# YuanchenBei/ColdRec

Hardware: AMD Instinct MI355X
Metric: ranked items/sec (full-catalogue eval) (higher is better)
Workload: dtype f32; 1 GPU; configs[3] full-catalogue eval: 1000000-row user table x 10000000 items, d=128, k=20, f32 tables, user block 131072 per step, rated CSR (mean ~50) + 20% cold-item bitmap ('warm' setting), item table row-sharded over 1 GPU(s); items=10000000, dim=128, k=20, parallelism=single GPU

## Files before the change

coldrec_amd/_lib.py:

```python
from __future__ import annotations

import ctypes
import os
import subprocess

_HERE = os.path.dirname(os.path.abspath(__file__))
LIB_PATH = os.environ.get("CRH_LIB") or os.path.join(_HERE, "lib", "libcoldrec_hip.so")
CSRC = os.path.join(_HERE, "csrc")

PAD_IDX = 0x7FFFFFFF
MASKED_SCORE = -1.0e9
MAX_K = 128

_lib = None

_vp, _i32, _i64, _sz, _f32 = ctypes.c_void_p, ctypes.c_int, ctypes.c_int64, ctypes.c_size_t, ctypes.c_float
_f64 = ctypes.c_double

SIGNATURES = {
    "crh_last_error": (ctypes.c_char_p, []),
    "crh_version": (_i32, []),
    "crh_score_topk_supports_dim": (_i32, [_i32]),
    "crh_score_topk_workspace_bytes": (_sz, [_i64, _i64, _i32, _i32]),
    "crh_score_topk_min_workspace_bytes": (_sz, [_i64, _i32]),
    "crh_score_topk_route": (_i32, [_i32, _i64, _i64, _i32, _i32, _sz, _i32, _i32, _vp, _vp]),
    "crh_score_topk_route_kernel": (ctypes.c_char_p, [_i32]),
    "crh_score_topk_screened": (_i32, [_i32, _i64, _i64, _i32, _i32, _sz, _i32, _i32]),
    "crh_score_topk_uncertified": (_i64, [_vp, _vp]),
    "crh_score_topk_screen_plan": (_i32, [_i64, _i64, _sz, _i32, _vp, _vp]),
    "crh_score_topk_screen_ordered": (_i32, [_i64, _i64, _sz, _i32]),
    "crh_score_topk_screen_map": (_i32, [_vp, _vp, _i64, _i64, _i64, _i32, _vp, _vp, _vp, _vp]),
    "crh_score_topk_screen_rated_tiles": (_i32, [_i64, _i64, _sz, _i32, _i32]),
    "crh_score_topk_screen_flags_bytes": (_sz, [_i64, _i64]),
    "crh_score_topk_screen_flags": (_i32, [_vp, _vp, _i64, _i64, _i64, _i32, _vp, _vp, _i64, _vp, _vp]),
    "crh_score_topk_f32": (_i32, [_vp, _vp, _i64, _vp, _i64, _i32, _vp, _vp, _vp, _i32, _i64, _vp, _vp,
                                  _vp, _sz, _vp]),
    "crh_score_topk_f32_ex": (_i32, [_vp, _vp, _i64, _vp, _i64, _i32, _vp, _vp, _vp, _i32, _i64, _vp, _vp,
                                     _vp, _sz, _vp, _i32, _vp, _vp]),
    "crh_score_screen_items_bytes": (_sz, [_i64, _i32]),
    "crh_score_screen_items_prepare": (_i32, [_vp, _i64, _i32, _vp, _i64, _i64, _vp, _sz, _vp, _sz, _vp, _vp]),
    "crh_score_screen_items_destroy": (_i32, [_vp]),
    "crh_score_topk_screen_item_preps": (_i64, []),
    "crh_score_topk_f32_prepared": (_i32, [_vp, _vp, _i64, _vp, _i64, _i32, _vp, _vp, _vp, _i32, _i64, _vp, _vp,
                                           _vp, _sz, _vp, _i32, _vp, _vp, _vp]),
    "crh_score_topk_f16_supports_dim": (_i32, [_i32]),
    "crh_score_topk_f16_workspace_bytes": (_sz, [_i64, _i64, _i32, _i32]),
    "crh_score_topk_f16_ex": (_i32, [_vp, _vp, _i64, _vp, _i64, _i32, _vp, _vp, _vp, _i32, _i64, _vp, _vp,
                                     _vp, _sz, _vp, _i32, _vp, _vp]),
    "crh_mask_topk_f32": (_i32, [_vp, _i64, _i64, _i64, _vp, _vp, _vp, _i32, _i64, _i32, _vp, _vp, _vp]),
    "crh_merge_topk": (_i32, [_vp, _vp, _i32, _i64, _i32, _i32, _vp, _vp, _vp]),
    "crh_bpr_workspace_bytes": (_sz, [_i64]),
    "crh_bpr_plan_ints": (_i64, [_i64]),
    "crh_bpr_heavy_threshold": (_i32, []),
    "crh_bpr_plan_build_host": (_i32, [_vp, _vp, _vp, _i64, _i64, _vp]),
    "crh_bpr_plan_build": (_i32, [_vp, _vp, _vp, _i64, _i64, _vp, _vp]),
    "crh_bpr_plan_build_large_workspace_bytes": (_sz, [_i64, _i64]),
    "crh_bpr_plan_build_large": (_i32, [_vp, _vp, _vp, _i64, _i64, _vp, _vp, _sz, _vp]),
    "crh_bpr_fwd_bwd_f32": (_i32, [_vp, _vp, _vp, _i32, _vp, _vp, _vp, _i64, _f32, _vp, _vp, _vp, _vp, _vp, _vp,
                                   _sz, _vp]),
    "crh_bpr_fwd_f32": (_i32, [_vp, _vp, _vp, _i32, _vp, _vp, _vp, _i64, _vp, _vp, _sz, _vp]),
    "crh_bpr_bwd_f32": (_i32, [_vp, _vp, _vp, _i32, _vp, _vp, _vp, _i64, _i64, _f32, _vp, _vp, _vp, _vp, _vp, _vp,
# ... 162 lines not shown
```

coldrec_amd/csrc/score_screen.hip:

```cpp
#include <math.h>

#include "score_topk_common.h"

#include <hipcub/device/device_radix_sort.hpp>

namespace crh_score {
namespace {

constexpr int SD = 128;
constexpr int FB_SCRATCH_SLICES = 64;

__device__ __forceinline__ float up_float(double x) {
    if (!(x <= 3.0e38)) return __builtin_inff();
    float f = (float)x;
    if ((double)f < x) f = __uint_as_float(__float_as_uint(f) + 1u);
    return f;
}

__device__ __forceinline__ int scale_exp(const unsigned* stats, int word) {
    const float m = __uint_as_float(stats[word]);
    if (!(m > 0.0f) || !(m <= 3.4e38f)) return 0;
    int E;
    frexpf(m, &E);
    return 15 - E;
}

__device__ __forceinline__ _Float16 to_f16(float x, int e) {
    const float y = ldexpf(x, e);
    _Float16 hv = (_Float16)y;
    if (fabsf((float)hv) < 6.103515625e-05f) hv = (_Float16)0.0f;
    return hv;
}

__device__ __forceinline__ float wave_max(float v) {
#pragma unroll
    for (int o = 32; o >= 1; o >>= 1) v = fmaxf(v, __shfl_xor(v, o));
    return v;
}

constexpr unsigned SCREEN_KEY_NONFINITE = 0x7F80u;
template <bool KEYS>
__global__ __launch_bounds__(256) void screen_maxabs_kernel(const float* __restrict__ tab, const int32_t* __restrict__ rows,
                                                            int64_t n_rows, unsigned* __restrict__ stats, int word,
                                                            uint16_t* __restrict__ keys) {
    const int64_t n4 = n_rows * (SD / 4);
    float m = 0.0f;
    for (int64_t e = (int64_t)blockIdx.x * 256 + threadIdx.x; e < n4; e += (int64_t)gridDim.x * 256) {
        const int64_t r = e / (SD / 4);
// ... 283 lines not shown
}

__global__ __launch_bounds__(256) void screen_certify_kernel(ScreenArgs s) {
    const int lane = threadIdx.x & 63;
    const int64_t slot = (int64_t)blockIdx.x * 4 + (threadIdx.x >> 6);
    if (slot >= s.n_users) return;
    const int KP = s.kp, K = s.k;
    const bool mine = lane < KP;
    int gi = CRH_PAD_IDX;
    float a = CRH_NEG_INF;
    if (mine) {
        gi = s.cand_idx[slot * KP + lane];
        a = s.cand_score[slot * KP + lane];
    }
    const bool real = mine && gi != CRH_PAD_IDX && (int64_t)gi >= s.item_base && (int64_t)gi < s.item_base + s.n_items;
    bool masked = false;
    if (real && s.bitmap) masked = (s.bitmap[gi >> 5] >> (gi & 31)) & 1u;
    if (real && !masked && s.rated_rowptr) masked = lane_in_list(s.rated_col, s.rated_rowptr[slot], s.rated_rowptr[slot + 1], gi);
    const int64_t urow = s.users ? (int64_t)s.users[slot] : slot;
    float sc = CRH_NEG_INF;
    if (real) sc = exact_chain(s.user_emb + urow * SD, s.item_emb + ((int64_t)gi - s.item_base) * SD);
    const bool ok = !mine || (real && !masked && __builtin_isfinite(a) && __builtin_isfinite(sc));
    int rank = 0;
    for (int j = 0; j < KP; ++j) {
        const float sj = __shfl(sc, j);
        const int ij = __shfl(gi, j);
        rank += (j != lane && crh_better(sj, ij, sc, gi)) ? 1 : 0;
    }
    const unsigned long long kth = __ballot(mine && rank == K - 1);
    const float ek = __shfl(sc, kth ? __builtin_ctzll(kth) : 0);
    const float a_last = __shfl(a, KP - 1);
    const float a_k = __shfl(a, K - 1);
    bool cert = s.mode != 3 && __ballot(!ok) == 0ull && kth != 0ull;
    if (cert) {
        const float* us = s.ustat + 3 * slot;
        const float R = __uint_as_float(s.stats[2]), N = __uint_as_float(s.stats[3]), Nh = __uint_as_float(s.stats[4]);
        const double B = screen_bound(us[0], us[1], us[2], R, N, Nh);
        const double unscale = ldexp(1.0, -(scale_exp(s.stats, 0) + scale_exp(s.stats, 1)));
        const double A = (double)a_last * unscale;
        double thr = A + B;
        thr += fabs(thr) * 0x1p-50;
        cert = (double)ek > thr && ek > CRH_MASKED_SCORE;
        const float Mk = __uint_as_float(s.stats[SCREEN_STAT_MARGIN]);
        if (Mk <= 3.4028235e38f) {
            double thr_m = ((double)a_k - (double)Mk) * unscale + B;
            thr_m += fabs(thr_m) * 0x1p-50;
            cert = cert && (double)ek > thr_m;
        }
    }
    if (cert) {
        if (mine && rank < K) {
            s.out_score[slot * K + rank] = sc;
            s.out_idx[slot * K + rank] = gi;
        }
    } else if (lane == 0) {
        const unsigned f = atomicAdd(s.stats + 5, 1u);
        s.fail_list[f] = (int32_t)slot;
    }
}

constexpr int64_t FB_WAVES = 2048 * 4;
constexpr int64_t FB_MIN_ITEMS = 1024;
constexpr int FB_FANIN = 64;
constexpr int FB_SLICES_MAX = FB_FANIN * FB_FANIN;
__device__ __forceinline__ int fb_slices(const ScreenArgs& s, int64_t count) {
    if (count <= 0) return 1;
    int64_t S = (FB_WAVES + count - 1) / count;
    const int64_t by_items = (s.n_items + FB_MIN_ITEMS - 1) / FB_MIN_ITEMS;
    const int64_t by_scratch = s.n_users * s.n_slices / count;
    if (S > by_items) S = by_items;
    if (S > by_scratch) S = by_scratch;
    if (S > FB_SLICES_MAX) S = FB_SLICES_MAX;
    return S < 1 ? 1 : (int)S;
}

__global__ __launch_bounds__(256) void screen_fallback_kernel(ScreenArgs s) {
    __shared__ float ush[4][SD];
    __shared__ float lsh[4][32];
    __shared__ int lih[4][32];
    __shared__ int cnth[4];
    const int lane = threadIdx.x & 63, wv = threadIdx.x >> 6;
    const int K = s.k;
    const int64_t count = s.stats[5];
    const int S = fb_slices(s, count);
    const int64_t n_work = count * S;
    float* ls = lsh[wv];
    int* li = lih[wv];
    int* cnt = &cnth[wv];
    for (int64_t w = (int64_t)blockIdx.x * 4 + wv; w < n_work; w += (int64_t)gridDim.x * 4) {
        const int64_t f = w / S;
        const int z = (int)(w % S);
        const int64_t slot = s.fail_list[f];
        const int64_t urow = s.users ? (int64_t)s.users[slot] : slot;
        ush[wv][lane] = s.user_emb[urow * SD + lane];
        ush[wv][lane + 64] = s.user_emb[urow * SD + lane + 64];
        if (lane == 0) *cnt = 0;
        const int64_t lo = s.n_items * z / S, hi = s.n_items * (z + 1) / S;
        float tau = CRH_NEG_INF;
        for (int64_t base = lo; base < hi; base += 64) {
            const int64_t i = base + lane;
            const bool valid = i < hi;
            const int gl = (int)(s.item_base + (valid ? i : lo));
            const bool bm = valid && s.bitmap && ((s.bitmap[gl >> 5] >> (gl & 31)) & 1u);
            float raw = CRH_NEG_INF;
            if (valid) {
                if (bm) {
                    raw = 0.0f;
#pragma unroll 8
                    for (int q = 0; q < SD; ++q) raw = __builtin_fmaf(ush[wv][q], 0.0f, raw);
                } else {
                    raw = exact_chain(ush[wv], s.item_emb + i * SD);
                }
            }
            unsigned long long cand = __ballot(valid && raw > tau);
            const unsigned long long bms = __ballot(bm);
            while (cand) {
                const int L = __builtin_ctzll(cand);
                cand &= cand - 1;
                float sc = __shfl(raw, L);
                const int g = (int)(s.item_base + base + L);
                const int n = __builtin_amdgcn_readfirstlane(*cnt);
                if (wave_list_rejects(ls, li, n, K, sc, g)) continue;
                bool masked = (bms >> L) & 1ull;
                if (!masked && s.rated_rowptr) masked = wave_is_masked(g, slot, s.rated_rowptr, s.rated_col, nullptr, lane);
                if (masked) sc = CRH_MASKED_SCORE;
                wave_list_insert(ls, li, cnt, K, sc, g, lane);
                tau = wave_list_tau(ls, __builtin_amdgcn_readfirstlane(*cnt), K);
            }
        }
        const int n = __builtin_amdgcn_readfirstlane(*cnt);
        const int64_t o = (f * S + z) * K;
        wave_list_store(ls, li, n, K, s.part_score + o, s.part_idx + o, lane);
    }
}

__global__ __launch_bounds__(256) void screen_fallback_merge_kernel(ScreenArgs s, int level) {
    __shared__ float lsh[4][32];
    __shared__ int lih[4][32];
    __shared__ int cnth[4];
    const int lane = threadIdx.x & 63, wv = threadIdx.x >> 6;
    const int K = s.k;
    const int64_t count = s.stats[5];
    const int S = fb_slices(s, count);
    const int last = S <= FB_FANIN ? 0 : 1;
    if (level > last) return;
    const int stride = level == 0 ? 1 : FB_FANIN;
    const int span = stride * FB_FANIN;
    const int G = (S + span - 1) / span;
    float* ls = lsh[wv];
    int* li = lih[wv];
    int* cnt = &cnth[wv];
    for (int64_t w = (int64_t)blockIdx.x * 4 + wv; w < count * G; w += (int64_t)gridDim.x * 4) {
        const int64_t f = w / G;
        const int z0 = (int)(w % G) * span;
        if (lane == 0) *cnt = 0;
        for (int z = z0; z < z0 + span && z < S; z += stride) {
            const int64_t o = (f * S + z) * K;
            const float es = lane < K ? s.part_score[o + lane] : CRH_NEG_INF;
            const int ei = lane < K ? s.part_idx[o + lane] : CRH_PAD_IDX;
            unsigned long long m = __ballot(lane < K && ei != CRH_PAD_IDX);
            while (m) {
                const int L = __builtin_ctzll(m);
                m &= m - 1;
                const float sc = __shfl(es, L);
                const int g = __shfl(ei, L);
                const int n = __builtin_amdgcn_readfirstlane(*cnt);
                if (n >= K && !crh_better(sc, g, ls[K - 1], li[K - 1])) break;
                wave_list_insert(ls, li, cnt, K, sc, g, lane);
            }
        }
        const int n = __builtin_amdgcn_readfirstlane(*cnt);
        if (level == last) {
            const int64_t slot = s.fail_list[f];
            wave_list_store(ls, li, n, K, s.out_score + slot * K, s.out_idx + slot * K, lane);
        } else {
            const int64_t o = (f * S + z0) * K;
            wave_list_store(ls, li, n, K, s.part_score + o, s.part_idx + o, lane);
        }
    }
}

}

int screen_fallback_slices(int64_t n_items) {
    const int64_t s = n_items / 4096;
    return (int)(s < 1 ? 1 : (s > FB_SCRATCH_SLICES ? FB_SCRATCH_SLICES : s));
}

size_t screen_scan_bytes(int64_t n_main) { return (size_t)((n_main + 31) / 32 / LIVE_WPB + 2) * sizeof(unsigned); }

int64_t screen_map_slots(int64_t n_main) { return ((n_main + 31) / 32 + 1) * 32; }

size_t screen_sort_bytes(int64_t n_slots) { return (size_t)n_slots * 8 + ((size_t)1 << 20); }

int launch_screen_map(const uint32_t* bitmap, int64_t item_base, int64_t n_items, int64_t prefix, unsigned* n_live, unsigned* scan,
                      int32_t* idmap, const ScreenOrder* ord, hipStream_t st) {
    const int64_t g0 = item_base + prefix, g1 = item_base + n_items;
    const int64_t n_words = ((g1 - 1) >> 5) - (g0 >> 5) + 1, nb = (n_words + LIVE_WPB - 1) / LIVE_WPB;
    hipLaunchKernelGGL(screen_live_count_kernel, dim3((unsigned)nb), dim3(256), 0, st, bitmap, g0, g1, scan);
    CRH_HIP(hipGetLastError());
    hipLaunchKernelGGL(screen_live_scan_kernel, dim3(1), dim3(256), 0, st, scan, nb, n_live);
    CRH_HIP(hipGetLastError());
    hipLaunchKernelGGL(screen_idmap_kernel, dim3((unsigned)nb), dim3(256), 0, st, bitmap, g0, g1, scan, idmap);
    CRH_HIP(hipGetLastError());
    if (ord == nullptr) return CRH_OK;
    const int64_t n_slots = screen_map_slots(n_items - prefix);
    hipLaunchKernelGGL(screen_sortkey_kernel, dim3((unsigned)((n_slots + 255) / 256)), dim3(256), 0, st, idmap, ord->rowkeys, n_live,
                       item_base, n_slots, ord->skeys_in);
    CRH_HIP(hipGetLastError());
    size_t need = 0;
    CRH_HIP(hipcub::DeviceRadixSort::SortPairs(nullptr, need, ord->skeys_in, ord->skeys_out, idmap, ord->idmap, (int)n_slots, 0, 16, st));
    if (need > ord->sort_tmp_bytes) {
        crh_set_error("screened route: the ordered map's sort asks for %zu bytes of temporary storage, %zu are reserved", need,
                      ord->sort_tmp_bytes);
        return CRH_ERR_WS;
    }
    need = ord->sort_tmp_bytes;
    CRH_HIP(hipcub::DeviceRadixSort::SortPairs(ord->sort_tmp, need, ord->skeys_in, ord->skeys_out, idmap, ord->idmap, (int)n_slots, 0, 16, st));
    return CRH_OK;
// ... 72 lines not shown
    int32_t* idmap = reinterpret_cast<int32_t*>(buf + o_map);
    int rc = CRH_OK;
    unsigned live = 0;
    hipError_t e = hipMemsetAsync(buf, 0, 256, st);
    if (e == hipSuccess) {
        hipLaunchKernelGGL(screen_maxabs_kernel<true>, dim3(2048), dim3(256), 0, st, item_emb, nullptr, n_items, stats, 0, ord.rowkeys);
        e = hipGetLastError();
    }
    if (e == hipSuccess) rc = launch_screen_map(bitmap, item_base, n_items, prefix, stats + SCREEN_STAT_LIVE, reinterpret_cast<unsigned*>(buf + o_scan), idmap, &ord, st);
    if (e == hipSuccess && rc == CRH_OK) {
        hipLaunchKernelGGL(screen_mapkeys_kernel, dim3((unsigned)((n_main + 255) / 256)), dim3(256), 0, st,
                           ordered ? ord.skeys_out : ord.skeys_in, n_main, keys_out);
        e = hipGetLastError();
    }
    if (e == hipSuccess && rc == CRH_OK)
        e = hipMemcpyAsync(map_out, ordered ? ord.idmap : idmap, (size_t)n_main * 4, hipMemcpyDeviceToDevice, st);
    if (e == hipSuccess && rc == CRH_OK && flags_out != nullptr) {
        int32_t* inv = reinterpret_cast<int32_t*>(buf + o_inv);
        rc = launch_screen_invmap(ordered ? ord.idmap : idmap, stats + SCREEN_STAT_LIVE, item_base + prefix, n_main, inv, st);
        if (rc == CRH_OK)
            rc = launch_screen_rated_tiles(rated_rowptr, rated_col, n_users, bitmap, item_base + prefix, item_base + n_items, inv, flags_out, st);
    }
    if (e == hipSuccess && rc == CRH_OK) e = hipMemcpyAsync(&live, stats + SCREEN_STAT_LIVE, 4, hipMemcpyDeviceToHost, st);
    if (e == hipSuccess) e = hipStreamSynchronize(st);
    (void)hipFree(buf);
    CRH_HIP(e);
    if (rc == CRH_OK) *count = (int64_t)live;
    return rc;
}

int launch_screen_certify(const ScreenArgs& s, hipStream_t st) {
    hipLaunchKernelGGL(screen_certify_kernel, dim3((unsigned)((s.n_users + 3) / 4)), dim3(256), 0, st, s);
    CRH_HIP(hipGetLastError());
    hipLaunchKernelGGL(screen_fallback_kernel, dim3((unsigned)(FB_WAVES / 4)), dim3(256), 0, st, s);
    CRH_HIP(hipGetLastError());
    for (int level = 0; level < 2; ++level) {
        hipLaunchKernelGGL(screen_fallback_merge_kernel, dim3(512), dim3(256), 0, st, s, level);
        CRH_HIP(hipGetLastError());
    }
    return CRH_OK;
}

}
```

coldrec_amd/csrc/score_topk.hip:

```cpp
#include <math.h>
#include <stdarg.h>
#include <stdlib.h>

#include <algorithm>
#include <atomic>
#include <vector>

#include "score_topk_common.h"

using namespace crh_score;

namespace {

__device__ __forceinline__ bool pack_row_masked(const uint32_t* bitmap, int64_t gid) {
    return bitmap != nullptr && ((bitmap[gid >> 5] >> (gid & 31)) & 1u);
}

template <int D>
__global__ __launch_bounds__(256) void pack_items_kernel(const float* __restrict__ v, int64_t n_items,
                                                         float* __restrict__ packed, const uint32_t* __restrict__ bitmap,
                                                         int64_t item_base) {
    constexpr int NCH = D / 8;
    __shared__ float tile[32][D + 4];
    const int64_t t = blockIdx.x;
// ... 1245 lines not shown
    const int32_t* stream_map = nullptr;
    if (compact) stream_map = reuse ? reinterpret_cast<const int32_t*>(prepared->buf + PL.map) : (ordered ? ord.idmap : idmap);
    _Float16* uh = reinterpret_cast<_Float16*>(ws + L.uh);
    float* seed_s = reinterpret_cast<float*>(ws + L.seed);
    int32_t* seed_i = reinterpret_cast<int32_t*>(seed_s + (size_t)n_users * KP);
    float* cand_s = reinterpret_cast<float*>(ws + L.cand);
    int32_t* cand_i = reinterpret_cast<int32_t*>(cand_s + (size_t)n_users * KP);
    char* scratch = ws + L.scratch;
    const size_t scratch_b = workspace_bytes - L.scratch;

    ScreenArgs s;
    s.user_emb = user_emb;
    s.users = users;
    s.n_users = n_users;
    s.item_emb = item_emb;
    s.n_items = n_items;
    s.item_base = item_base;
    s.rated_rowptr = rated_rowptr;
    s.rated_col = rated_col;
    s.bitmap = cand_bitmap;
    s.k = k;
    s.kp = KP;
    s.mode = screen_mode();
    s.cand_score = cand_s;
    s.cand_idx = cand_i;
    s.stats = reinterpret_cast<unsigned*>(ws + L.stats);
    s.ustat = reinterpret_cast<float*>(ws + L.ustat);
    s.fail_list = reinterpret_cast<int32_t*>(ws + L.fail);
    s.n_slices = screen_fallback_slices(n_items);
    s.part_score = reinterpret_cast<float*>(scratch);
    s.part_idx = reinterpret_cast<int32_t*>(s.part_score + (size_t)n_users * s.n_slices * k);
    s.out_score = out_score;
    s.out_idx = out_idx;

    int rc = CRH_OK;
    if (reuse) {
        CRH_HIP(hipMemcpyAsync(s.stats, prepared->buf + PL.stats, 256, hipMemcpyDeviceToDevice, st));
    } else {
        CRH_HIP(hipMemsetAsync(s.stats, 0, 256, st));
        rc = screen_items_build(s, s.stats, pk, P, idmap, reinterpret_cast<unsigned*>(ws + L.scan), ordered ? &ord : nullptr, tbits, st);
        if (rc != CRH_OK) return rc;
    }
    const char* margin_env = getenv("CRH_SCORE_SCREEN_MARGIN");
    rc = launch_screen_prep_users(s, uh, !(margin_env && atoi(margin_env) == 0), st);
    if (rc != CRH_OK) return rc;
    if (ev_kernel_start) CRH_HIP(hipEventRecord(reinterpret_cast<hipEvent_t>(ev_kernel_start), st));

    ScoreArgs a = {};
    a.user_emb = uh;
    a.n_users = n_users;
    a.rated_rowptr = rated_rowptr;
    a.rated_col = rated_col;
    a.bitmap = cand_bitmap;
    a.k = KP;
    a.tile_bits = reinterpret_cast<const uint32_t*>(pk);
    if (P > 0) {
        const int64_t stride = P;
        const int upw_pw = users_per_wave(2, D);
        int64_t chunk = (int64_t)(scratch_b / ((size_t)stride * sizeof(float))) & ~(int64_t)63;
        if (chunk > n_users) chunk = n_users;
        a.packed = pk;
        a.n_items = P;
        a.item_base = item_base;
        a.dense = reinterpret_cast<float*>(scratch);
        a.dense_stride = stride;
        for (int64_t u0 = 0; u0 < n_users; u0 += chunk) {
// ... 235 lines not shown
    p->n_items = n_items;
    p->item_base = item_base;
    p->prefix = P;
    p->d = d;
    p->bitmap = cand_bitmap;
    p->compact = compact;
    p->ordered = ordered;
    p->stream = st;
    p->buf = buf;
    *handle = p;
    return CRH_OK;
}

extern "C" int crh_score_screen_items_destroy(void* handle) {
    if (handle == nullptr) return CRH_OK;
    ScreenItems* p = reinterpret_cast<ScreenItems*>(handle);
    CRH_CHECK_ARG(p->magic == SCREEN_ITEMS_MAGIC, "crh_score_screen_items_destroy: not a prepared-items handle");
    p->magic = 0;
    delete p;
    return CRH_OK;
}

extern "C" int64_t crh_score_topk_screen_item_preps(void) { return screen_item_preps.load(std::memory_order_relaxed); }

extern "C" int64_t crh_score_topk_uncertified(const void* workspace, void* stream) {
    CRH_CHECK_ARG(workspace != nullptr, "crh_score_topk_uncertified: NULL workspace");
    unsigned n = 0;
    hipStream_t st = reinterpret_cast<hipStream_t>(stream);
    CRH_HIP(hipMemcpyAsync(&n, reinterpret_cast<const unsigned*>(workspace) + 5, sizeof(n), hipMemcpyDeviceToHost, st));
    CRH_HIP(hipStreamSynchronize(st));
    return (int64_t)n;
}

extern "C" const char* crh_score_topk_route_kernel(int route) {
    switch (route & 15) {
        case CRH_ROUTE_DENSE: return "score_topk_kernel";
        case CRH_ROUTE_FUSED_WAVE: return "score_topk_kernel";
        case CRH_ROUTE_FUSED_WG: return "score_topk_wg_kernel";
        case CRH_ROUTE_FUSED_DMA: return "score_topk_dma_kernel";
        default: return "";
    }
}

extern "C" int crh_score_topk_f32_ex(const float* user_emb, const int32_t* users, int64_t n_users,
                                     const float* item_emb, int64_t n_items, int d,
                                     const int64_t* rated_rowptr, const int32_t* rated_col,
                                     const uint32_t* cand_bitmap, int k, int64_t item_base,
                                     float* out_score, int32_t* out_idx, void* workspace,
                                     size_t workspace_bytes, void* stream, int n_splits,
                                     void* ev_kernel_start, void* ev_kernel_stop) {
    return score_topk_any(4, user_emb, users, n_users, item_emb, n_items, d, rated_rowptr, rated_col, cand_bitmap, k,
                          item_base, out_score, out_idx, workspace, workspace_bytes, stream, n_splits,
                          ev_kernel_start, ev_kernel_stop, "crh_score_topk_f32");
}

extern "C" int crh_score_topk_f32_prepared(const float* user_emb, const int32_t* users, int64_t n_users,
                                           const float* item_emb, int64_t n_items, int d,
                                           const int64_t* rated_rowptr, const int32_t* rated_col,
                                           const uint32_t* cand_bitmap, int k, int64_t item_base,
                                           float* out_score, int32_t* out_idx, void* workspace,
                                           size_t workspace_bytes, void* stream, int n_splits,
                                           void* ev_kernel_start, void* ev_kernel_stop, const void* prepared) {
    return score_topk_any(4, user_emb, users, n_users, item_emb, n_items, d, rated_rowptr, rated_col, cand_bitmap, k,
                          item_base, out_score, out_idx, workspace, workspace_bytes, stream, n_splits,
                          ev_kernel_start, ev_kernel_stop, "crh_score_topk_f32", reinterpret_cast<const ScreenItems*>(prepared));
}
// ... 24 lines not shown
```

coldrec_amd/csrc/score_topk_common.h:

```cpp
#pragma once
#include <math.h>

#include "crh_common.h"
#include "topk_list.h"

namespace crh_score {

struct ScoreArgs {
    const void* user_emb;
    const int32_t* users;
    int64_t n_users;
    const void* item_emb;
    const void* packed;
    int64_t n_items;
    const int64_t* rated_rowptr;
    const int32_t* rated_col;
    const uint32_t* bitmap;
    int k;
    int64_t item_base;
    int n_splits;
    int64_t n_ugroups;
    float* out_score;
    int32_t* out_idx;
    int ablate;
    unsigned long long* wave_clock;
    unsigned* xcd_sync;
    int sync_window;
    int64_t sync_stride;
    float* dense;
    int64_t dense_stride;
    int64_t user_base;
    const float* seed_score;
    const int32_t* seed_idx;
    const uint32_t* tile_bits;
    const int32_t* idmap;
    const unsigned* n_live;
// ... 279 lines not shown
    return __builtin_amdgcn_readfirstlane((int)ok) != 0;
}

constexpr int WG_RING = 3;

constexpr int SCREEN_KP = 28;
__attribute__((visibility("hidden"))) int launch_score_dma(int esz, int d, int mode, const ScoreArgs& a, hipStream_t stream);
__attribute__((visibility("hidden"))) size_t score_dma_lds_bytes(int row_bytes, int k, int ring_slots, bool flags, bool compact = false);
__attribute__((visibility("hidden"))) int score_dma_ring_slots(int esz, int d, int k, int mode);

struct ScreenArgs {
    const float* user_emb;
    const int32_t* users;
    int64_t n_users;
    const float* item_emb;
    int64_t n_items;
    int64_t item_base;
    const int64_t* rated_rowptr;
    const int32_t* rated_col;
    const uint32_t* bitmap;
    int k;
    int kp;
    int mode;
    const float* cand_score;
    const int32_t* cand_idx;
    unsigned* stats;
    float* ustat;
    int32_t* fail_list;
    float* part_score;
    int32_t* part_idx;
    int n_slices;
    float* out_score;
    int32_t* out_idx;
};
__attribute__((visibility("hidden"))) int screen_fallback_slices(int64_t n_items);
constexpr int SCREEN_STAT_LIVE = 6;
constexpr int SCREEN_STAT_MAXB = 7;
constexpr int SCREEN_STAT_MARGIN = 8;
__attribute__((visibility("hidden"))) size_t screen_scan_bytes(int64_t n_main);
struct ScreenOrder {
    uint16_t* rowkeys;
    uint16_t* skeys_in;
    uint16_t* skeys_out;
    int32_t* idmap;
    void* sort_tmp;
    size_t sort_tmp_bytes;
};
__attribute__((visibility("hidden"))) int64_t screen_map_slots(int64_t n_main);
__attribute__((visibility("hidden"))) size_t screen_sort_bytes(int64_t n_slots);
__attribute__((visibility("hidden"))) int launch_screen_prep_items(const ScreenArgs& s, unsigned* stats, _Float16* packed, int64_t prefix,
                                                                   int32_t* idmap, unsigned* scan, const ScreenOrder* ord, hipStream_t st);
__attribute__((visibility("hidden"))) int launch_screen_prep_users(const ScreenArgs& s, _Float16* uh, int margin_on, hipStream_t st);
__attribute__((visibility("hidden"))) int screen_map_only(const uint32_t* bitmap, const float* item_emb, int64_t n_items,
                                                          int64_t item_base, int64_t prefix, int ordered, int32_t* map_out,
                                                          int32_t* keys_out, int64_t* count, hipStream_t st,
                                                          const int64_t* rated_rowptr = nullptr, const int32_t* rated_col = nullptr,
                                                          int64_t n_users = 0, uint32_t* flags_out = nullptr);
__attribute__((visibility("hidden"))) int launch_screen_invmap(const int32_t* map, const unsigned* n_live, int64_t g0, int64_t n_main,
                                                               int32_t* inv, hipStream_t st);
__attribute__((visibility("hidden"))) size_t screen_rated_tiles_bytes(int64_t n_users, int64_t n_main);
__attribute__((visibility("hidden"))) int launch_screen_rated_tiles(const int64_t* rated_rowptr, const int32_t* rated_col, int64_t n_users,
                                                                    const uint32_t* bitmap, int64_t g0, int64_t g1, const int32_t* inv,
                                                                    uint32_t* flags, hipStream_t st);
__attribute__((visibility("hidden"))) int launch_screen_certify(const ScreenArgs& s, hipStream_t st);

}
```

coldrec_amd/ops.py:

```python
from __future__ import annotations

import ctypes
import weakref
import os
from typing import Optional, Tuple

import numpy as np
import torch

from . import _lib

SUPPORTED_DIMS = (8, 16, 32, 64, 128, 256)
SUPPORTED_DIMS_F16 = (16, 32, 64, 128, 256)


def _need_cuda(*ts):
    for t in ts:
        if t is not None and not t.is_cuda:
            raise RuntimeError("coldrec_amd ops need tensors on the MI355X (cuda device); there is no CPU path")


def pad_dim(table: torch.Tensor) -> torch.Tensor:
    d = table.shape[1]
    dims = SUPPORTED_DIMS_F16 if table.dtype == torch.float16 else SUPPORTED_DIMS
# ... 205 lines not shown


def score_topk_screen_rated_tiles(n_users: int, n_items: int, d: int, k: int, has_bitmap: bool = True, has_rated: bool = True) -> bool:
    return bool(_lib.lib().crh_score_topk_screen_rated_tiles(n_users, n_items, _score_ws_bytes(n_users, n_items, d, k),
                                                             1 if has_bitmap else 0, 1 if has_rated else 0))


def score_topk_screen_flags(cand_bitmap: torch.Tensor, item_emb: torch.Tensor, rated_rowptr: torch.Tensor, rated_col: torch.Tensor,
                            item_base: int = 0, prefix: int = 0, ordered: bool = True) -> torch.Tensor:
    _need_cuda(cand_bitmap, item_emb, rated_rowptr, rated_col)
    assert cand_bitmap.dtype == torch.int32 and item_emb.dtype == torch.float32 and item_emb.shape[1] == 128
    assert rated_rowptr.dtype == torch.int64 and rated_col.dtype == torch.int32
    item_emb = item_emb.contiguous()
    n_users, n_main = rated_rowptr.shape[0] - 1, item_emb.shape[0] - prefix
    L = _lib.lib()
    groups = ((n_users + 127) // 128 + 3) // 4
    words = int(L.crh_score_topk_screen_flags_bytes(n_users, n_main)) // 4
    out = torch.empty((groups, words // groups), dtype=torch.int32, device=item_emb.device)
    rc = L.crh_score_topk_screen_flags(_lib.ptr(cand_bitmap), _lib.ptr(item_emb), item_emb.shape[0], item_base, prefix,
                                       1 if ordered else 0, _lib.ptr(rated_rowptr), _lib.ptr(rated_col), n_users, _lib.ptr(out),
                                       _lib.current_stream())
    _lib.check(rc, "crh_score_topk_screen_flags")
    return out


def score_topk_uncertified(device=None) -> int:
    dev = torch.device("cuda", torch.cuda.current_device()) if device is None else torch.device(device)
    key = (dev.type, dev.index, torch.cuda.current_stream(dev).cuda_stream)
    buf = _ws_cache.get(key)
    if buf is None:
        raise RuntimeError("score_topk_uncertified: no scoring workspace on this stream")
    n = _lib.lib().crh_score_topk_uncertified(_lib.ptr(buf), _lib.current_stream())
    _lib.check(n if n < 0 else 0, "crh_score_topk_uncertified")
    return int(n)


def mask_topk(scores: torch.Tensor, k: int, rated_rowptr=None, rated_col=None, cand_bitmap=None,
              item_base: int = 0, write_back: bool = True):
    _need_cuda(scores, rated_rowptr, rated_col, cand_bitmap)
    assert scores.dtype == torch.float32 and scores.dim() == 2 and scores.stride(1) == 1
    n_users, n_items = scores.shape
    dev = scores.device
    out = (torch.empty((n_users, k), dtype=torch.float32, device=dev),
           torch.empty((n_users, k), dtype=torch.int32, device=dev))
    rc = _lib.lib().crh_mask_topk_f32(_lib.ptr(scores), n_users, n_items, scores.stride(0),
                                      _lib.ptr(rated_rowptr), _lib.ptr(rated_col), _lib.ptr(cand_bitmap), k,
                                      item_base, 1 if write_back else 0, _lib.ptr(out[0]), _lib.ptr(out[1]),
                                      _lib.current_stream())
    _lib.check(rc, "crh_mask_topk_f32")
    return out


def merge_topk(scores: torch.Tensor, idx: torch.Tensor, k_out: int):
    _need_cuda(scores, idx)
    assert scores.dtype == torch.float32 and idx.dtype == torch.int32
    scores, idx = scores.contiguous(), idx.contiguous()
    n_lists, n_users, k_in = scores.shape
    dev = scores.device
    out = (torch.empty((n_users, k_out), dtype=torch.float32, device=dev),
           torch.empty((n_users, k_out), dtype=torch.int32, device=dev))
    rc = _lib.lib().crh_merge_topk(_lib.ptr(scores), _lib.ptr(idx), n_lists, n_users, k_in, k_out,
                                   _lib.ptr(out[0]), _lib.ptr(out[1]), _lib.current_stream())
    _lib.check(rc, "crh_merge_topk")
    return out


# ... 1328 lines not shown
```

include/coldrec_hip.h:

```cpp
#ifndef COLDREC_HIP_H
#define COLDREC_HIP_H

#include <stddef.h>
#include <stdint.h>

#ifdef __cplusplus
extern "C" {
#endif

#define CRH_OK 0
#define CRH_ERR_ARG (-1)
#define CRH_ERR_HIP (-2)
#define CRH_ERR_WS (-3)
#define CRH_PAD_IDX 0x7fffffff
#define CRH_MASKED_SCORE (-1.0e9f)
#define CRH_MAX_K 128

const char* crh_last_error(void);
int crh_version(void);
int crh_score_topk_supports_dim(int d);

size_t crh_score_topk_workspace_bytes(int64_t n_users, int64_t n_items, int d, int k);
size_t crh_score_topk_min_workspace_bytes(int64_t n_users, int k);

#define CRH_ROUTE_DENSE 1
#define CRH_ROUTE_FUSED_WAVE 2
#define CRH_ROUTE_FUSED_WG 3
#define CRH_ROUTE_FUSED_DMA 4
#define CRH_ROUTE_SEEDED 16
#define CRH_ROUTE_DMA_FLAGS 32
int crh_score_topk_route(int elem_bytes, int64_t n_users, int64_t n_items, int d, int k, size_t workspace_bytes,
                         int has_bitmap, int n_splits, int64_t* prefix_items, int* picked_splits);
const char* crh_score_topk_route_kernel(int route);
int crh_score_topk_screen_plan(int64_t n_users, int64_t n_items, size_t workspace_bytes, int has_bitmap, int* cuts, int* compact);
int crh_score_topk_screen_ordered(int64_t n_users, int64_t n_items, size_t workspace_bytes, int has_bitmap);
int crh_score_topk_screen_map(const uint32_t* bitmap, const float* item_emb, int64_t n_items, int64_t item_base, int64_t prefix,
                              int ordered, int32_t* map_out, int32_t* keys_out, int64_t* count, void* stream);
int crh_score_topk_screen_rated_tiles(int64_t n_users, int64_t n_items, size_t workspace_bytes, int has_bitmap, int has_rated);
size_t crh_score_topk_screen_flags_bytes(int64_t n_users, int64_t n_main);
int crh_score_topk_screen_flags(const uint32_t* bitmap, const float* item_emb, int64_t n_items, int64_t item_base, int64_t prefix,
                                int ordered, const int64_t* rated_rowptr, const int32_t* rated_col, int64_t n_users,
                                uint32_t* flags_out, void* stream);
int crh_score_topk_screened(int elem_bytes, int64_t n_users, int64_t n_items, int d, int k, size_t workspace_bytes,
                            int has_bitmap, int n_splits);
int64_t crh_score_topk_uncertified(const void* workspace, void* stream);
size_t crh_score_screen_items_bytes(int64_t n_items, int has_bitmap);
int crh_score_screen_items_prepare(const float* item_emb, int64_t n_items, int d, const uint32_t* cand_bitmap, int64_t item_base,
                                   int64_t n_users, void* items_buf, size_t items_bytes, void* workspace, size_t workspace_bytes,
                                   void* stream, void** handle);
int crh_score_screen_items_destroy(void* handle);
int64_t crh_score_topk_screen_item_preps(void);
int crh_score_topk_f32_prepared(const float* user_emb, const int32_t* users, int64_t n_users,
                                const float* item_emb, int64_t n_items, int d,
                                const int64_t* rated_rowptr, const int32_t* rated_col,
                                const uint32_t* cand_bitmap, int k, int64_t item_base,
                                float* out_score, int32_t* out_idx, void* workspace,
                                size_t workspace_bytes, void* stream, int n_splits,
                                void* ev_kernel_start, void* ev_kernel_stop, const void* prepared);
int crh_score_topk_f32(const float* user_emb, const int32_t* users, int64_t n_users,
                       const float* item_emb, int64_t n_items, int d,
                       const int64_t* rated_rowptr, const int32_t* rated_col,
                       const uint32_t* cand_bitmap, int k, int64_t item_base,
                       float* out_score, int32_t* out_idx,
                       void* workspace, size_t workspace_bytes, void* stream);

int crh_score_topk_f32_ex(const float* user_emb, const int32_t* users, int64_t n_users,
                          const float* item_emb, int64_t n_items, int d,
                          const int64_t* rated_rowptr, const int32_t* rated_col,
                          const uint32_t* cand_bitmap, int k, int64_t item_base,
                          float* out_score, int32_t* out_idx,
                          void* workspace, size_t workspace_bytes, void* stream, int n_splits,
                          void* ev_kernel_start, void* ev_kernel_stop);

int crh_score_topk_f16_supports_dim(int d);
size_t crh_score_topk_f16_workspace_bytes(int64_t n_users, int64_t n_items, int d, int k);
int crh_score_topk_f16_ex(const void* user_emb, const int32_t* users, int64_t n_users,
                          const void* item_emb, int64_t n_items, int d,
                          const int64_t* rated_rowptr, const int32_t* rated_col,
// ... 296 lines not shown
```

Measured before the change: 6722 billion items/s.

## Add windowed re-screen stage for uncertified users before exact fallback

Users whose screened top-k cannot be certified are routed into a new window stage first. It rescans the packed f16 item table once per chunk of up to 64 users, collects candidate rows that fall inside a per-user bound window, and then scores those candidates exactly and ranks them. Only users whose window overflows or holds fewer than k valid items still go to the expensive per-user full-catalogue fallback. This adds two kernel launches and an extra pass over the packed items, in exchange for sending fewer users down the fallback path.

Result: no change. 6778 billion items/s (median of 6 runs) (+0.8%).

```diff
diff --git a/coldrec_amd/_lib.py b/coldrec_amd/_lib.py
--- a/coldrec_amd/_lib.py
+++ b/coldrec_amd/_lib.py
@@ -27,6 +27,8 @@
     "crh_score_topk_route_kernel": (ctypes.c_char_p, [_i32]),
     "crh_score_topk_screened": (_i32, [_i32, _i64, _i64, _i32, _i32, _sz, _i32, _i32]),
     "crh_score_topk_uncertified": (_i64, [_vp, _vp]),
+    "crh_score_topk_window_answered": (_i64, [_vp, _vp]),
+    "crh_score_topk_screen_window_users": (_i64, [_i64, _i64, _i32, _sz, _i32, _i32]),
     "crh_score_topk_screen_plan": (_i32, [_i64, _i64, _sz, _i32, _vp, _vp]),
     "crh_score_topk_screen_ordered": (_i32, [_i64, _i64, _sz, _i32]),
     "crh_score_topk_screen_map": (_i32, [_vp, _vp, _i64, _i64, _i64, _i32, _vp, _vp, _vp, _vp]),
diff --git a/coldrec_amd/csrc/score_screen.hip b/coldrec_amd/csrc/score_screen.hip
--- a/coldrec_amd/csrc/score_screen.hip
+++ b/coldrec_amd/csrc/score_screen.hip
@@ -8,12 +8,17 @@
 namespace {
 
 constexpr int SD = 128;
-constexpr int FB_SCRATCH_SLICES = 64;
 
 __device__ __forceinline__ float up_float(double x) {
     if (!(x <= 3.0e38)) return __builtin_inff();
     float f = (float)x;
     if ((double)f < x) f = __uint_as_float(__float_as_uint(f) + 1u);
+    return f;
+}
+
+__device__ __forceinline__ float down_float(double x) {
+    float f = (float)x;
+    if ((double)f > x) f = nextafterf(f, -__builtin_inff());
     return f;
 }
 
@@ -363,6 +368,7 @@
     const float a_last = __shfl(a, KP - 1);
     const float a_k = __shfl(a, K - 1);
     bool cert = s.mode != 3 && __ballot(!ok) == 0ull && kth != 0ull;
+    double wd = __builtin_nan(""), w1d = wd, w2d = wd;
     if (cert) {
         const float* us = s.ustat + 3 * slot;
         const float R = __uint_as_float(s.stats[2]), N = __uint_as_float(s.stats[3]), Nh = __uint_as_float(s.stats[4]);
@@ -371,6 +377,13 @@
         const double A = (double)a_last * unscale;
         double thr = A + B;
         thr += fabs(thr) * 0x1p-50;
+        const int e0 = scale_exp(s.stats, 0), e1 = scale_exp(s.stats, 1);
+        wd = ((double)ek - B) * ldexp(1.0, e0 + e1);
+        const double gd = SD * 0x1p-24 / (1.0 - SD * 0x1p-24), gp = 0x1p-12;
+        const double c1 = ((double)us[0] * R * (1.0 + gd) + 0x1p-126) * (1.0 + 0x1p-20);
+        const double c2 = ((double)us[2] + gd * (double)us[0] + gp * (double)us[1]) * (1.0 + 0x1p-20);
+        w1d = ((double)ek - c1) * ldexp(1.0, e0 + e1);
+        w2d = c2 * ldexp(1.0, e1);
         cert = (double)ek > thr && ek > CRH_MASKED_SCORE;
         const float Mk = __uint_as_float(s.stats[SCREEN_STAT_MARGIN]);
         if (Mk <= 3.4028235e38f) {
@@ -387,6 +400,139 @@
     } else if (lane == 0) {
         const unsigned f = atomicAdd(s.stats + 5, 1u);
         s.fail_list[f] = (int32_t)slot;
+    }
+    if (s.win_mode == 0 || lane != 0) return;
+    bool to_win = (!cert || s.win_mode == 2) && ek > CRH_MASKED_SCORE && fabs(wd) <= 3.0e38 && fabs(w1d) <= 3.0e38 &&
+                  w2d <= 1.0e38;
+    if (to_win) {
+        const unsigned p = atomicAdd(s.stats + SCREEN_STAT_WIN, 1u);
+        to_win = p < (unsigned)s.win_cap;
+        if (to_win) {
+            s.win_list[p] = (int32_t)slot;
+            s.win_w[3 * p + 0] = down_float(wd);
+            s.win_w[3 * p + 1] = down_float(w1d - fabs(w1d) * 0x1p-20 - 0x1p-100);
+            s.win_w[3 * p + 2] = up_float(w2d * (1.0 + 0x1p-20));
+            s.win_cnt[p] = 0u;
+        }
+    }
+    if (!to_win && !cert) s.fail2[atomicAdd(s.stats + SCREEN_STAT_FAIL2, 1u)] = (int32_t)slot;
+}
+
+constexpr int WIN_CHUNK = 64;
+__device__ __forceinline__ int window_users(const ScreenArgs& s) {
+    const unsigned n = s.stats[SCREEN_STAT_WIN];
+    return (int)(n < (unsigned)s.win_cap ? n : (unsigned)s.win_cap);
+}
+__global__ __launch_bounds__(256) void screen_window_scan_kernel(ScreenArgs s) {
+    __shared__ __attribute__((aligned(16))) float ush[WIN_CHUNK][SD];
+    __shared__ float wsh[WIN_CHUNK][3];
+    const int n_win = window_users(s);
+    if (n_win == 0) return;
+    const int lane = threadIdx.x & 63, wv = threadIdx.x >> 6, r = lane & 31, h = lane >> 5;
+    const int64_t TP = s.prefix >> 5;
+    const int64_t rows_main = s.stream_map ? (int64_t)s.stats[SCREEN_STAT_LIVE] : s.n_items - s.prefix;
+    const int64_t T = TP + ((rows_main + 31) >> 5);
+    const u32x4* src = reinterpret_cast<const u32x4*>(s.packed);
+    for (int c0 = 0; c0 < n_win; c0 += WIN_CHUNK) {
+        const int nc = n_win - c0 < WIN_CHUNK ? n_win - c0 : WIN_CHUNK;
+        __syncthreads();
+        for (int x = threadIdx.x; x < nc * SD; x += 256)
+            ush[x / SD][x % SD] = (float)s.uh[(int64_t)s.win_list[c0 + x / SD] * SD + x % SD];
+        for (int x = threadIdx.x; x < 3 * nc; x += 256) wsh[x / 3][x % 3] = s.win_w[3 * c0 + x];
+        __syncthreads();
+        for (int64_t t = (int64_t)blockIdx.x * 4 + wv; t < T; t += (int64_t)gridDim.x * 4) {
+            float v[64];
+#pragma unroll
+            for (int j = 0; j < 8; ++j) {
+                const f16x8 x = __builtin_bit_cast(f16x8, src[(t * 8 + j) * 64 + lane]);
+#pragma unroll
+                for (int c = 0; c < 8; ++c) v[8 * j + c] = (float)x[c];
+            }
+            float vn = 0.0f;
+#pragma unroll
+            for (int c = 0; c < 64; ++c) vn = __builtin_fmaf(v[c], v[c], vn);
+            vn += __shfl_xor(vn, 32);
+            vn = sqrtf(vn) * (1.0f + 0x1p-12f);
+            const int64_t row = (t << 5) + r, q = row - s.prefix;
+            const bool live = t < TP || q < rows_main;
+            int gi = (int)(s.item_base + row);
+            if (t >= TP && s.stream_map) gi = live ? s.stream_map[q] : CRH_PAD_IDX;
+            for (int u = 0; u < nc; ++u) {
+                float a = 0.0f;
+#pragma unroll
+                for (int j = 0; j < 8; ++j) {
+                    const f32x4 u0 = *reinterpret_cast<const f32x4*>(&ush[u][16 * j + 8 * h]);
+                    const f32x4 u1 = *reinterpret_cast<const f32x4*>(&ush[u][16 * j + 8 * h + 4]);
+#pragma unroll
+                    for (int c = 0; c < 4; ++c) a = __builtin_fmaf(u0[c], v[8 * j + c], a);
+#pragma unroll
+                    for (int c = 0; c < 4; ++c) a = __builtin_fmaf(u1[c], v[8 * j + 4 + c], a);
+                }
+                a += __shfl_xor(a, 32);
+                if (h == 0 && live && a >= wsh[u][0] && __builtin_fmaf(wsh[u][2], vn, a) >= wsh[u][1]) {
+                    const unsigned p = atomicAdd(s.win_cnt + c0 + u, 1u);
+                    if (p < (unsigned)SCREEN_WIN_ROWS) s.win_buf[(int64_t)(c0 + u) * SCREEN_WIN_ROWS + p] = gi;
+                }
+            }
+        }
+    }
+}
+
+__global__ __launch_bounds__(256) void screen_window_finish_kernel(ScreenArgs s) {
+    const int n_win = window_users(s);
+    const int lane = threadIdx.x & 63, K = s.k;
+    for (int64_t f = (int64_t)blockIdx.x * 4 + (threadIdx.x >> 6); f < n_win; f += (int64_t)gridDim.x * 4) {
+        const int64_t slot = s.win_list[f];
+        const unsigned cnt = s.win_cnt[f];
+        bool good = cnt <= (unsigned)SCREEN_WIN_ROWS;
+        float sc[4];
+        int gi[4];
+        if (good) {
+            const int64_t urow = s.users ? (int64_t)s.users[slot] : slot;
+            int n_valid = 0;
+#pragma unroll
+            for (int q = 0; q < 4; ++q) {
+                const unsigned e = 64u * q + lane;
+                sc[q] = CRH_NEG_INF;
+                gi[q] = CRH_PAD_IDX;
+                if (e < cnt) {
+                    const int g = s.win_buf[f * SCREEN_WIN_ROWS + e];
+                    bool masked = s.bitmap && ((s.bitmap[g >> 5] >> (g & 31)) & 1u);
+                    if (!masked && s.rated_rowptr) masked = lane_in_list(s.rated_col, s.rated_rowptr[slot], s.rated_rowptr[slot + 1], g);
+                    if (!masked) {
+                        gi[q] = g;
+                        sc[q] = exact_chain(s.user_emb + urow * SD, s.item_emb + ((int64_t)g - s.item_base) * SD);
+                    }
+                }
+                n_valid += __popcll(__ballot(gi[q] != CRH_PAD_IDX));
+                if (__ballot(gi[q] != CRH_PAD_IDX && !__builtin_isfinite(sc[q])) != 0ull) good = false;
+            }
+            good = good && n_valid >= K;
+        }
+        if (!good) {
+            if (lane == 0) s.fail2[atomicAdd(s.stats + SCREEN_STAT_FAIL2, 1u)] = (int32_t)slot;
+            continue;
+        }
+        int rank[4] = {0, 0, 0, 0};
+        for (unsigned e0 = 0; e0 < cnt; e0 += 64) {
+            const int q2 = (int)(e0 >> 6);
+            const float sq = q2 == 0 ? sc[0] : q2 == 1 ? sc[1] : q2 == 2 ? sc[2] : sc[3];
+            const int iq = q2 == 0 ? gi[0] : q2 == 1 ? gi[1] : q2 == 2 ? gi[2] : gi[3];
+            for (int j = 0; j < 64; ++j) {
+                const float sj = __shfl(sq, j);
+                const int ij = __shfl(iq, j);
+                if (ij == CRH_PAD_IDX) continue;
+#pragma unroll
+                for (int q = 0; q < 4; ++q) rank[q] += crh_better(sj, ij, sc[q], gi[q]) ? 1 : 0;
+            }
+        }
+#pragma unroll
+        for (int q = 0; q < 4; ++q)
+            if (gi[q] != CRH_PAD_IDX && rank[q] < K) {
+                s.out_score[slot * K + rank[q]] = sc[q];
+                s.out_idx[slot * K + rank[q]] = gi[q];
+            }
+        if (lane == 0) atomicAdd(s.stats + SCREEN_STAT_WIN_DONE, 1u);
     }
 }
 
@@ -412,7 +558,7 @@
     __shared__ int cnth[4];
     const int lane = threadIdx.x & 63, wv = threadIdx.x >> 6;
     const int K = s.k;
-    const int64_t count = s.stats[5];
+    const int64_t count = *s.fb_count;
     const int S = fb_slices(s, count);
     const int64_t n_work = count * S;
     float* ls = lsh[wv];
@@ -421,7 +567,7 @@
     for (int64_t w = (int64_t)blockIdx.x * 4 + wv; w < n_work; w += (int64_t)gridDim.x * 4) {
         const int64_t f = w / S;
         const int z = (int)(w % S);
-        const int64_t slot = s.fail_list[f];
+        const int64_t slot = s.fb_list[f];
         const int64_t urow = s.users ? (int64_t)s.users[slot] : slot;
         ush[wv][lane] = s.user_emb[urow * SD + lane];
         ush[wv][lane + 64] = s.user_emb[urow * SD + lane + 64];
@@ -471,7 +617,7 @@
     __shared__ int cnth[4];
     const int lane = threadIdx.x & 63, wv = threadIdx.x >> 6;
     const int K = s.k;
-    const int64_t count = s.stats[5];
+    const int64_t count = *s.fb_count;
     const int S = fb_slices(s, count);
     const int last = S <= FB_FANIN ? 0 : 1;
     if (level > last) return;
@@ -502,7 +648,7 @@
         }
         const int n = __builtin_amdgcn_readfirstlane(*cnt);
         if (level == last) {
-            const int64_t slot = s.fail_list[f];
+            const int64_t slot = s.fb_list[f];
             wave_list_store(ls, li, n, K, s.out_score + slot * K, s.out_idx + slot * K, lane);
         } else {
             const int64_t o = (f * S + z0) * K;
@@ -511,11 +657,6 @@
     }
 }
 
-}
-
-int screen_fallback_slices(int64_t n_items) {
-    const int64_t s = n_items / 4096;
-    return (int)(s < 1 ? 1 : (s > FB_SCRATCH_SLICES ? FB_SCRATCH_SLICES : s));
 }
 
 size_t screen_scan_bytes(int64_t n_main) { return (size_t)((n_main + 31) / 32 / LIVE_WPB + 2) * sizeof(unsigned); }
@@ -654,6 +795,12 @@
 int launch_screen_certify(const ScreenArgs& s, hipStream_t st) {
     hipLaunchKernelGGL(screen_certify_kernel, dim3((unsigned)((s.n_users + 3) / 4)), dim3(256), 0, st, s);
     CRH_HIP(hipGetLastError());
+    if (s.win_mode != 0) {
+        hipLaunchKernelGGL(screen_window_scan_kernel, dim3(2048), dim3(256), 0, st, s);
+        CRH_HIP(hipGetLastError());
+        hipLaunchKernelGGL(screen_window_finish_kernel, dim3(64), dim3(256), 0, st, s);
+        CRH_HIP(hipGetLastError());
+    }
     hipLaunchKernelGGL(screen_fallback_kernel, dim3((unsigned)(FB_WAVES / 4)), dim3(256), 0, st, s);
     CRH_HIP(hipGetLastError());
     for (int level = 0; level < 2; ++level) {
diff --git a/coldrec_amd/csrc/score_topk.hip b/coldrec_amd/csrc/score_topk.hip
--- a/coldrec_amd/csrc/score_topk.hip
+++ b/coldrec_amd/csrc/score_topk.hip
@@ -1301,6 +1301,23 @@
     s.part_idx = reinterpret_cast<int32_t*>(s.part_score + (size_t)n_users * s.n_slices * k);
     s.out_score = out_score;
     s.out_idx = out_idx;
+    const char* win_env = getenv("CRH_SCORE_SCREEN_WINDOW");
+    const int win_req = s.mode == 3 ? 0 : (win_env ? atoi(win_env) : 1);
+    const ScreenWindowPlan wp = screen_window_plan(n_users, s.n_slices, k, scratch_b, win_req < 0 || win_req > 2 ? 0 : win_req);
+    s.win_mode = wp.cap > 0 ? win_req : 0;
+    s.win_cap = (int)wp.cap;
+    auto win_at = [&](size_t o) { return wp.cap > 0 ? scratch + wp.base + o : nullptr; };
+    s.fail2 = reinterpret_cast<int32_t*>(win_at(wp.W.fail2));
+    s.win_list = reinterpret_cast<int32_t*>(win_at(wp.W.win_list));
+    s.win_w = reinterpret_cast<float*>(win_at(wp.W.win_w));
+    s.win_cnt = reinterpret_cast<unsigned*>(win_at(wp.W.win_cnt));
+    s.win_buf = reinterpret_cast<int32_t*>(win_at(wp.W.win_buf));
+    s.fb_list = s.win_mode ? s.fail2 : s.fail_list;
+    s.fb_count = s.win_mode ? s.stats + SCREEN_STAT_FAIL2 : s.stats + 5;
+    s.uh = uh;
+    s.packed = pk;
+    s.stream_map = stream_map;
+    s.prefix = P;
 
     int rc = CRH_OK;
     if (reuse) {
@@ -1602,6 +1619,25 @@
     return (int64_t)n;
 }
 
+extern "C" int64_t crh_score_topk_screen_window_users(int64_t n_users, int64_t n_items, int k, size_t workspace_bytes, int has_bitmap,
+                                                      int has_rated) {
+    if (n_users <= 0 || n_items <= 0 || k < 1) return 0;
+    const ScreenPlan plan = plan_screen(n_users, n_items, workspace_bytes, has_bitmap != 0, has_rated != 0);
+    if (workspace_bytes < plan.L.need) return 0;
+    const char* e = getenv("CRH_SCORE_SCREEN_WINDOW");
+    const int req = screen_mode() == 3 ? 0 : (e ? atoi(e) : 1);
+    return screen_window_plan(n_users, screen_fallback_slices(n_items), k, workspace_bytes - plan.L.scratch, req < 0 || req > 2 ? 0 : req).cap;
+}
+
+extern "C" int64_t crh_score_topk_window_answered(const void* workspace, void* stream) {
+    CRH_CHECK_ARG(workspace != nullptr, "crh_score_topk_window_answered: NULL workspace");
+    unsigned n = 0;
+    hipStream_t st = reinterpret_cast<hipStream_t>(stream);
+    CRH_HIP(hipMemcpyAsync(&n, reinterpret_cast<const unsigned*>(workspace) + SCREEN_STAT_WIN_DONE, sizeof(n), hipMemcpyDeviceToHost, st));
+    CRH_HIP(hipStreamSynchronize(st));
+    return (int64_t)n;
+}
+
 extern "C" const char* crh_score_topk_route_kernel(int route) {
     switch (route & 15) {
         case CRH_ROUTE_DENSE: return "score_topk_kernel";
diff --git a/coldrec_amd/csrc/score_topk_common.h b/coldrec_amd/csrc/score_topk_common.h
--- a/coldrec_amd/csrc/score_topk_common.h
+++ b/coldrec_amd/csrc/score_topk_common.h
@@ -2,6 +2,7 @@
 #include <math.h>
 
 #include "crh_common.h"
+#include "screen_window_layout.h"
 #include "topk_list.h"
 
 namespace crh_score {
@@ -347,8 +348,23 @@
     int n_slices;
     float* out_score;
     int32_t* out_idx;
-};
-__attribute__((visibility("hidden"))) int screen_fallback_slices(int64_t n_items);
+    const int32_t* fb_list;
+    const unsigned* fb_count;
+    int win_mode;
+    int win_cap;
+    int32_t* win_list;
+    float* win_w;
+    unsigned* win_cnt;
+    int32_t* win_buf;
+    int32_t* fail2;
+    const _Float16* uh;
+    const _Float16* packed;
+    const int32_t* stream_map;
+    int64_t prefix;
+};
+constexpr int SCREEN_STAT_WIN = 9;
+constexpr int SCREEN_STAT_FAIL2 = 10;
+constexpr int SCREEN_STAT_WIN_DONE = 11;
 constexpr int SCREEN_STAT_LIVE = 6;
 constexpr int SCREEN_STAT_MAXB = 7;
 constexpr int SCREEN_STAT_MARGIN = 8;
diff --git a/coldrec_amd/csrc/screen_window_layout.h b/coldrec_amd/csrc/screen_window_layout.h
--- /dev/null
+++ b/coldrec_amd/csrc/screen_window_layout.h
@@ -0,0 +1,56 @@
+#pragma once
+#include <stddef.h>
+#include <stdint.h>
+
+namespace crh_score {
+
+constexpr int SCREEN_WIN_ROWS = 256;
+constexpr int SCREEN_WIN_USERS_MAX = 256;
+
+constexpr int FB_SCRATCH_SLICES = 64;
+inline int screen_fallback_slices(int64_t n_items) {
+    const int64_t s = n_items / 4096;
+    return (int)(s < 1 ? 1 : (s > FB_SCRATCH_SLICES ? FB_SCRATCH_SLICES : s));
+}
+
+struct ScreenWindowLayout {
+    size_t fail2, win_list, win_w, win_cnt, win_buf, need;
+};
+inline ScreenWindowLayout screen_window_layout(int64_t n_users, int64_t cap) {
+    auto al = [](size_t x) { return (x + 255) & ~(size_t)255; };
+    ScreenWindowLayout W;
+    W.fail2 = 0;
+    W.win_list = W.fail2 + al((size_t)n_users * sizeof(int32_t));
+    W.win_w = W.win_list + al((size_t)cap * sizeof(int32_t));
+    W.win_cnt = W.win_w + al((size_t)cap * 3 * sizeof(float));
+    W.win_buf = W.win_cnt + al((size_t)cap * sizeof(unsigned));
+    W.need = W.win_buf + al((size_t)cap * SCREEN_WIN_ROWS * sizeof(int32_t));
+    return W;
+}
+
+struct ScreenWindowPlan {
+    int64_t cap;
+    size_t base;
+    ScreenWindowLayout W;
+};
+inline ScreenWindowPlan screen_window_plan(int64_t n_users, int n_slices, int k, size_t scratch_b, int mode) {
+    ScreenWindowPlan p;
+    p.cap = 0;
+    p.base = (((size_t)n_users * (size_t)n_slices * (size_t)k * 8) + 255) & ~(size_t)255;
+    p.W = screen_window_layout(n_users, 0);
+    if (mode <= 0 || n_users <= 0 || p.base > scratch_b) return p;
+    const size_t room = scratch_b - p.base;
+    const int64_t small = n_users < SCREEN_WIN_USERS_MAX ? n_users : SCREEN_WIN_USERS_MAX;
+    const int64_t tries[2] = {mode >= 2 ? n_users : small, small};
+    for (int q = 0; q < 2; ++q) {
+        const ScreenWindowLayout W = screen_window_layout(n_users, tries[q]);
+        if (W.need <= room) {
+            p.cap = tries[q];
+            p.W = W;
+            return p;
+        }
+    }
+    return p;
+}
+
+}
diff --git a/coldrec_amd/ops.py b/coldrec_amd/ops.py
--- a/coldrec_amd/ops.py
+++ b/coldrec_amd/ops.py
@@ -261,6 +261,17 @@
         raise RuntimeError("score_topk_uncertified: no scoring workspace on this stream")
     n = _lib.lib().crh_score_topk_uncertified(_lib.ptr(buf), _lib.current_stream())
     _lib.check(n if n < 0 else 0, "crh_score_topk_uncertified")
+    return int(n)
+
+
+def score_topk_window_answered(device=None) -> int:
+    dev = torch.device("cuda", torch.cuda.current_device()) if device is None else torch.device(device)
+    key = (dev.type, dev.index, torch.cuda.current_stream(dev).cuda_stream)
+    buf = _ws_cache.get(key)
+    if buf is None:
+        raise RuntimeError("score_topk_window_answered: no scoring workspace on this stream")
+    n = _lib.lib().crh_score_topk_window_answered(_lib.ptr(buf), _lib.current_stream())
+    _lib.check(n if n < 0 else 0, "crh_score_topk_window_answered")
     return int(n)
 
 
diff --git a/include/coldrec_hip.h b/include/coldrec_hip.h
--- a/include/coldrec_hip.h
+++ b/include/coldrec_hip.h
@@ -44,6 +44,8 @@
 int crh_score_topk_screened(int elem_bytes, int64_t n_users, int64_t n_items, int d, int k, size_t workspace_bytes,
                             int has_bitmap, int n_splits);
 int64_t crh_score_topk_uncertified(const void* workspace, void* stream);
+int64_t crh_score_topk_window_answered(const void* workspace, void* stream);
+int64_t crh_score_topk_screen_window_users(int64_t n_users, int64_t n_items, int k, size_t workspace_bytes, int has_bitmap, int has_rated);
 size_t crh_score_screen_items_bytes(int64_t n_items, int has_bitmap);
 int crh_score_screen_items_prepare(const float* item_emb, int64_t n_items, int d, const uint32_t* cand_bitmap, int64_t item_base,
                                    int64_t n_users, void* items_buf, size_t items_bytes, void* workspace, size_t workspace_bytes,
```
